# owl-project/owlExaBrick

Measured on AMD Instinct MI355X. Metric: frames/sec at 2048^2 DVR, exajet-like, MI355X, higher is better.
Workload: dtype f32; 1 GPU; c4_exajet (seed 0xe7a0003 procedural AMR, scale 1.0): 640512000 cells / 1251000 bricks / 13349488 regions, 2048x2048 DVR, dt 0.5, alpha ramp, gradient shading on, space skipping on, frameID 0; tiling=16x16 tiles interleaved over 1 GPU(s)

## Files before the change

owlexabrick_amd/csrc/exa_kernels.hip:

```cpp
#include "exa_device.h"
#include <cfloat>
#include <type_traits>

#if EXA_BASIS_FORM == 0 && EXA_EMPTY_CELLS
#define EXA_FORM_NS form0e
#elif EXA_BASIS_FORM == 0
#define EXA_FORM_NS form0
#elif EXA_BASIS_FORM == 1 && EXA_EMPTY_CELLS
#error "empty cells are a per-corner property: the per-axis association (EXA_BASIS_FORM 1) does not apply"
#elif EXA_BASIS_FORM == 1
#define EXA_FORM_NS form1
#else
#error "EXA_BASIS_FORM is 0 (source order) or 1 (per-axis association with fused multiply-adds)"
#endif
#define EXA_F1 (EXA_BASIS_FORM == 1)
#ifndef EXA_TU_ROPE
#define EXA_TU_ROPE 0
#endif
#ifndef EXA_TU_SAMPLE
#define EXA_TU_SAMPLE 0
#endif
#ifndef EXA_TU_STREAM
#define EXA_TU_STREAM 0
#endif
// ... 1818 lines not shown
  rnd.state = __float_as_uint(baseRnd.w);
  if (j & 1u) { rnd.next(); rnd.next(); }
  const V3 wN = mk(ngAmb.x, ngAmb.y, ngAmb.z);
  const V3 vN = fabsf(wN.x) > fabsf(wN.y) ? normalize(mk(-wN.z, 0.f, wN.x)) : normalize(mk(0.f, wN.z, -wN.y));
  const V3 uN = cross(vN, wN);
  const float u1 = rnd.next(), u2 = rnd.next();
  const float rr = sqrtf(u1);
  const float theta = 2.f * 3.14159265358979323846f * u2;
  const V3 sp = mk(rr * cosf(theta), rr * sinf(theta), sqrtf(1.f - u1));
  Ray ao_ray;
  ao_ray.org = mk(posFd.x, posFd.y, posFd.z);
  ao_ray.dir = normalize((sp.x * uN + sp.y * vN) + sp.z * wN);
  ao_ray.tmin = 1e-4f; ao_ray.tmax = fs.ao.length;
  return ao_ray;
}

enum { kAoDirClasses = 24, kAoCellShift = 5 };
__device__ __forceinline__ uint32_t aoRayKey(const RenderArgs &a, uint32_t slot, V3 d)
{
  const float ax = fabsf(d.x), ay = fabsf(d.y), az = fabsf(d.z);
  const uint32_t dom = (ax >= ay && ax >= az) ? 0u : (ay >= az ? 1u : 2u);
  const uint32_t oct = (d.x < 0.f ? 1u : 0u) | (d.y < 0.f ? 2u : 0u) | (d.z < 0.f ? 4u : 0u);
  uint32_t cell;
  if (a.world == 1) {
    const uint32_t px = slot % (uint32_t)a.W, py = slot / (uint32_t)a.W;
    cell = (py >> kAoCellShift) * (((uint32_t)a.W + 31u) >> kAoCellShift) + (px >> kAoCellShift);
  } else {
    cell = slot >> 10;
  }
  return cell * kAoDirClasses + oct * 3u + dom;
}
#if !EXA_TU_ROPE
__global__ __launch_bounds__(256) void aoKeyKernel(const RenderArgs a)
{
  const unsigned numRays = 2u * a.aoCount[0];
  for (unsigned j = blockIdx.x * 256u + threadIdx.x; j < numRays; j += gridDim.x * 256u) {
    const AoRecord *r = a.aoRecs + (j >> 1);
    const Ray ray = aoRayOf(a.fs, r->posFd, r->ngAmb, r->baseRnd, j);
    const uint32_t key = min(aoRayKey(a, r->slot, ray.dir), a.aoBins - 1u);
    a.aoKeys[j] = key;
    atomicAdd(&a.aoHist[key], 1u);
  }
}
__global__ __launch_bounds__(1024) void aoScanKernel(uint32_t *hist, uint32_t numBins)
{
  __shared__ uint32_t part[1024];
  const uint32_t per = (numBins + 1023u) / 1024u;
  const uint32_t b0 = min(threadIdx.x * per, numBins), b1 = min(b0 + per, numBins);
  uint32_t sum = 0;
  for (uint32_t b = b0; b < b1; b++) sum += hist[b];
  part[threadIdx.x] = sum;
  __syncthreads();
  for (uint32_t off = 1; off < 1024u; off <<= 1) {
    const uint32_t v = threadIdx.x >= off ? part[threadIdx.x - off] : 0u;
    __syncthreads();
    part[threadIdx.x] += v;
    __syncthreads();
  }
  uint32_t run = part[threadIdx.x] - sum;
  for (uint32_t b = b0; b < b1; b++) { const uint32_t c = hist[b]; hist[b] = run; run += c; }
}
__global__ __launch_bounds__(256) void aoScatterKernel(const RenderArgs a)
{
  const unsigned numRays = 2u * a.aoCount[0];
  for (unsigned j = blockIdx.x * 256u + threadIdx.x; j < numRays; j += gridDim.x * 256u)
    a.aoOrder[atomicAdd(&a.aoHist[a.aoKeys[j]], 1u)] = j;
}
__global__ __launch_bounds__(256) void aoFinalizeKernel(const RenderArgs a)
{
  const unsigned numHits = a.aoCount[0];
  for (unsigned h = blockIdx.x * 256u + threadIdx.x; h < numHits; h += gridDim.x * 256u) {
    const AoRecord *r = a.aoRecs + h;
    const float4 posFd = r->posFd, ngAmb = r->ngAmb, baseRnd = r->baseRnd;
    const uint32_t slot = r->slot;
    const int hitCnt = (int)a.aoHit[2u * h] + (int)a.aoHit[2u * h + 1u];
    const float shadow = (float)hitCnt / 2;
    const float fd = posFd.w;
    const float ns = 1.f - shadow;
    const float t_hit = a.surf[slot].w;
    a.surf[slot] = make_float4(ngAmb.w + baseRnd.x * fd * ns, ngAmb.w + baseRnd.y * fd * ns, ngAmb.w + baseRnd.z * fd * ns, t_hit);
  }
}

#endif

template <bool ISO_ONLY, bool SORTED>
__global__ __launch_bounds__(kKdBlock, (ISO_ONLY ? EXA_AO_ISO_WAVES : EXA_PREPASS_WAVES)) void aoRaysKdKernel(const RenderArgs a)
{
  static_assert(ldsFits(kdLds(1), ISO_ONLY ? EXA_AO_ISO_WAVES : EXA_PREPASS_WAVES), "LDS per workgroup x waves per SIMD exceeds the CU's 160 KB");
  const LdsPtrs lds = carveLds(kdLds(a.numXfChannels));
  Ctx<0> C;
  kernelPrologue(C, a, lds);
  float *stackF = lds.stackF, *qT = lds.qT;
  int *qRegion = lds.qRegion;
  C.fastSampler = a.fastSampler != 0;
  const ExaHipFrameState &fs = a.fs;
  const unsigned numRays = 2u * a.aoCount[0];
  for (;;) {
    unsigned base = 0;
    if ((threadIdx.x & 63) == 0) base = atomicAdd(&a.aoCount[2], 64u);
    base = (unsigned)__shfl((int)base, 0, 64);
    if (base >= numRays) break;
    const unsigned k = base + (threadIdx.x & 63);
    const bool live = k < numRays;
    const unsigned j = (SORTED && live) ? a.aoOrder[k] : k;
    int hitFlag = 0;
    float4 posFd = make_float4(0.f, 0.f, 0.f, 0.f), ngAmb = posFd, baseRnd = posFd;
    uint32_t slot = 0;
    if (live) {
      const AoRecord *r = a.aoRecs + (j >> 1);
      posFd = r->posFd; ngAmb = r->ngAmb; baseRnd = r->baseRnd; slot = r->slot;
      const Ray ao_ray = aoRayOf(fs, posFd, ngAmb, baseRnd, j);
      SurfaceHit ao;
      traceSurfacesKd<0, ISO_ONLY>(C, ao_ray, ao, false, stackF, qRegion, qT);
      if (ao.primID >= 0 || ao.primID == EXA_PRIMID_ISOSURFACE || ao.primID == EXA_PRIMID_PLANE
          || ao.primID == EXA_PRIMID_STREAMLINE) hitFlag = 1;
      if (SORTED) a.aoHit[j] = (uint8_t)hitFlag;
    }
    if (SORTED) continue;
    const int other = __shfl_xor(hitFlag, 1, 64);
    if (live && !(j & 1u)) {
      const int hitCnt = hitFlag + other;
      const float shadow = (float)hitCnt / 2;
      const float fd = posFd.w;
      const float ns = 1.f - shadow;
      const float t_hit = a.surf[slot].w;
      a.surf[slot] = make_float4(ngAmb.w + baseRnd.x * fd * ns, ngAmb.w + baseRnd.y * fd * ns, ngAmb.w + baseRnd.z * fd * ns, t_hit);
    }
  }
  if (C.guardTripped) atomicExch(a.errorFlag, 1);
}

constexpr int marchWaves(int MULTI, int STATS, bool SMALL, int NCH, bool ROPE)
{
  return NCH > 1 ? (NCH == 2 ? EXA_IL2_WAVES : EXA_IL34_WAVES)
             : (MULTI == 1 ? EXA_MULTI_WAVES
                           : (MULTI ? 5 : ((ROPE && !STATS && SMALL && EXA_BASIS_FORM == 1) ? EXA_ROPE_WAVES : EXA_MARCH_WAVES)));
}

template <bool GRAD, bool FAST, int MULTI, bool SURF, int STATS, bool SMALL, int NCH = 0, bool ROPE = false>
__global__ __launch_bounds__(kKdBlock, marchWaves(MULTI, STATS, SMALL, NCH, ROPE)) void renderFrameKdKernel(const RenderArgs a)
{
  constexpr bool CUBE = NCH == 1;
  constexpr int IL = CUBE ? 0 : NCH;
  static_assert(!CUBE || (MULTI == 0 && ROPE && SMALL && STATS == 0 && EXA_BASIS_FORM == 1 && !EXA_EMPTY_CELLS),
                "the cube records are a variant of the shipped one-channel 32-bit rope march");
#ifndef EXA_CUBE_LEAN
#define EXA_CUBE_LEAN 0
#endif
#ifndef EXA_MARCH_DEFER
#define EXA_MARCH_DEFER 1
#endif
  constexpr bool DEFER = CUBE && EXA_MARCH_DEFER;
  constexpr bool LEAN = marchWaves(MULTI, STATS, SMALL, NCH, ROPE) >= 7 && (!CUBE || EXA_CUBE_LEAN || (DEFER && GRAD));
  constexpr int PACKED_CT = !ROPE ? -1 : (STATS == 1 ? 0 : (SMALL ? 1 : -1));
  const bool packedRec = PACKED_CT < 0 ? a.leafBeginBits != 0 : PACKED_CT != 0;
  static_assert(IL == 0 || (MULTI == 2 && STATS == 0), "the interleaved march is a multi-channel variant of the shipped kernel");
  constexpr int KS = marchLds(MULTI == 1, false, 0).stackEntries;
  constexpr int QN = marchLds(MULTI == 1, ROPE, 0).queueEntries;
  static_assert(ldsFits(marchLds(MULTI == 1, ROPE, IL ? IL : (MULTI ? 2 : 1)), marchWaves(MULTI, STATS, SMALL, NCH, ROPE)),
                "LDS per workgroup x waves per SIMD exceeds the CU's 160 KB: shorten the queue or lower the occupancy");
  const LdsPtrs lds = carveLds(marchLds(MULTI == 1, ROPE, a.numXfChannels));
  float4 *queue4 = lds.queue4;
  float *stackF = lds.stackF, *qT = lds.qT;
  int *qRegion = lds.qRegion;
  for (int i = threadIdx.x; i < a.numXfChannels * EXA_NUM_XF_VALUES; i += kKdBlock) lds.xf[i] = a.xf[i];
  __syncthreads();
  Ctx<STATS> C;
  initCtx(C, a, lds);
  const unsigned long long clockBegin = clock64();
  if (STATS) for (int i = 0; i < ST_COUNT; i++) C.st[i] = 0;
  __shared__ unsigned long long lapMarks[STATS == 2 ? 8 * (kKdBlock / 64) : 1];
  if (STATS == 2) {
    C.lapMark = lapMarks + 8 * (threadIdx.x >> 6);
    if ((threadIdx.x & 63) == 0) {
      C.lapMark[0] = clock64(); C.lapMark[1] = ST_T_OTHER - ST_T_BRICK;
      for (int i = 2; i < 7; i++) C.lapMark[i] = 0;
    }
  }

  const int wavesPerBlock = kKdBlock / 64;
  const int gwave = blockIdx.x * wavesPerBlock + (threadIdx.x >> 6);
  const int tile = a.tileMap[gwave >> 2];
  const int tx = tile % a.tilesX, ty = tile / a.tilesX;
  const int wave = gwave & 3, lane = threadIdx.x & 63;
  const int inX = ((wave & 1) << 3) + laneX(lane), inY = ((wave >> 1) << 3) + laneY(lane);
  const int px = tx * kTile + inX, py = ty * kTile + inY;
  const bool inside = px < a.W && py < a.H && (a.debugPixel < 0 || a.debugPixel == px + a.W * py);

  if (STATS == 1 && a.walkProbe) C.probe = a.walkProbe + size_t(gwave) * kWalkProbeSize;
  unsigned marchIters = 0;
  if (inside) {
    const ExaHipFrameState &fs = a.fs;
    const int frameID = fs.frameID;
    Lcg rnd;
    Ray ray = cameraRay(a, px, py, rnd);
    float surface_t_hit = ray.tmax;
    if (SURF) {
      const size_t slot0 = slotOf(a, tile, inX, inY, px, py);
      surface_t_hit = a.surf[slot0].w;
      rnd.state = a.surfRnd[slot0];
    }
    const float interleavedSamplingOffset = rnd.next();
    clipToVoxelSpace(fs, ray, surface_t_hit);
    ray.org.x = __int_as_float(__builtin_amdgcn_readfirstlane(__float_as_int(ray.org.x)));
    ray.org.y = __int_as_float(__builtin_amdgcn_readfirstlane(__float_as_int(ray.org.y)));
    ray.org.z = __int_as_float(__builtin_amdgcn_readfirstlane(__float_as_int(ray.org.z)));

    Color4 pixelColor; pixelColor.x = pixelColor.y = pixelColor.z = pixelColor.w = 0.f;
    const int numChannels = a.p.numPrimaryChannels;

    KdWalk w;
    w.pk.v = 0;
    {
      Ray whole = ray; whole.tmin = -INFINITY; whole.tmax = INFINITY;
      float r0, r1;
      const bool hit = boxTest(whole, mk(a.kdLo), mk(a.kdHi), r0, r1);
      w.tn = fmaxf(r0, ray.tmin);
      w.tf = fminf(r1, ray.tmax);
      w.tEnd = w.tf;
      w.ref = (hit && w.tn < w.tf) ? (ROPE ? a.ropeRoot : a.kdMarchRoot) : EXA_KD_DONE;
    }
    bool ropeFast = false;
    if (ROPE) ropeFast = a.ropeFastDiv != 0 && !anyLane(!ropeRayInRange(ray));

    float walkTmin = ray.tmin;

    bool haveSeg = false;
    int listBegin = 0, listSize = 0;
    float flcw = 1.f;
    float t1 = 0.f, t_i = 0.f, t_sample = 0.f, actual_dt = 0.f;
    int child = 0, chan = 0;
    int4 hb0 = make_int4(0, 0, 0, 1), hb1 = make_int4(1, 1, 1, 0);
    Basis B;
    B.sumWV = 0.f; B.sumW = 0.f; B.sumD = mk(0.f, 0.f, 0.f); B.sumDC = mk(0.f, 0.f, 0.f);
    float xWV[IL > 1 ? IL - 1 : 1];
    V3 xD[IL > 1 ? IL - 1 : 1];
#pragma unroll
    for (int c = 0; c < (IL > 1 ? IL - 1 : 1); c++) { xWV[c] = 0.f; xD[c] = mk(0.f, 0.f, 0.f); }
    const float *field0 = a.sc.scalars + a.sc.channelOffset[0];
    const float *field = field0;
    float xfRcpRange0 = 0.f, xfRange0 = 0.f;
    if (FAST && !MULTI) {
      xfRange0 = __int_as_float(__builtin_amdgcn_readfirstlane(__float_as_int((fs.xfDomain[0][1] - fs.xfDomain[0][0]) + 1e-20f)));
      xfRcpRange0 = __int_as_float(__builtin_amdgcn_readfirstlane(__float_as_int(__builtin_amdgcn_rcpf(xfRange0))));
    }
    float xfRcpRangeN[IL ? IL : 1], xfRangeN[IL ? IL : 1];
#pragma unroll
    for (int c = 0; c < (IL ? IL : 1); c++) {
      xfRangeN[c] = (FAST && IL) ? __int_as_float(__builtin_amdgcn_readfirstlane(__float_as_int((fs.xfDomain[c][1] - fs.xfDomain[c][0]) + 1e-20f))) : 0.f;
      xfRcpRangeN[c] = (FAST && IL) ? __int_as_float(__builtin_amdgcn_readfirstlane(__float_as_int(__builtin_amdgcn_rcpf(xfRangeN[c])))) : 0.f;
    }

    bool pending = false;
    float pendDt = 0.f, pendFlcw = 1.f;
    auto shadePending = [&]() {
      if (B.sumW > 1e-20f) {
        const float cellValue = fdivExact<FAST>(B.sumWV, B.sumW);
        V3 grad = mk(0.f, 0.f, 0.f);
        if (GRAD) grad = gradOf(B.sumW, B.sumWV, B.sumD, B.sumDC);
        integrateVolume<FAST, STATS, (FAST && !MULTI), LEAN>(C, ray, pixelColor, pendDt, cellValue, grad, pendFlcw, 0, xfRcpRange0, xfRange0);
      }
      B.sumWV = 0.f; B.sumW = 0.f; B.sumD = mk(0.f, 0.f, 0.f); B.sumDC = mk(0.f, 0.f, 0.f);
      pending = false;
    };

    unsigned iter = 0;
    for (;; iter++) {
      if (iter == 0xfffffff0u) { C.guardTripped = true; break; }
      if (anyLane(!haveSeg && w.pk.get(PK_QCOUNT) == 0 && w.ref != EXA_KD_DONE)) {
        C.lap(ST_T_WALK);
        do {
          const bool want = w.pk.get(PK_QCOUNT) < QN && w.ref != EXA_KD_DONE;
          if (want) {
            if (ROPE) ropeStep<STATS, SMALL, QN, LEAN, PACKED_CT>(C, w, walkTmin, a, queue4, ray, ropeFast, interleavedSamplingOffset);
            else kdStep<false, STATS, SMALL, KS>(C, w, walkTmin, a, stackF, qRegion, qT, ray, 0, walkTmin, 1.f, a.kdMarchNodes, a.kdMarchRoot);
          }
        } while (anyLane(!haveSeg && w.pk.get(PK_QCOUNT) == 0 && w.ref != EXA_KD_DONE));
      }
      if (!haveSeg) {
        C.lap(ST_T_SEG);
        const int qc = w.pk.get(PK_QCOUNT);
        if (qc == 0) break;
        const int qh = w.pk.get(PK_QHEAD);
        int region;
        float t0, tiQueued = 0.f;
        if (ROPE) {
          const float4 e = queue4[qh * kKdBlock];
          region = __float_as_int(e.x); t1 = e.y; tiQueued = e.z; t0 = e.w;
        } else {
          region = qRegion[qh * kKdBlock];
          t0 = qT[(2 * qh) * kKdBlock];
          t1 = qT[(2 * qh + 1) * kKdBlock];
        }
        w.pk.template incWrap<QN>(PK_QHEAD);
        w.pk.dec(PK_QCOUNT);
        if (packedRec) {
          const unsigned d = (unsigned)region;
          listBegin = (int)(d & ((1u << a.leafBeginBits) - 1u));
          listSize = (int)((d >> a.leafBeginBits) & ((1u << a.leafSizeBits) - 1u)) + 1;
          flcw = __int_as_float((127 + (int)(d >> (a.leafBeginBits + a.leafSizeBits))) << 23);
        } else {
          const RegionInfo ri = a.sc.regionInfo[region];
          listBegin = ri.listBegin; listSize = ri.listSize;
          flcw = ri.finestLevelCellWidth;
        }
        C.count(ST_SEGMENTS);
        haveSeg = true;
        w.pk.setBit(PK_NEEDHDR);
        if (ROPE && packedRec)
          t_i = tiQueued;
        else if (a.invDtPow2 != 0.f)
          t_i = firstSampleTPow2(t0, a.p.dt * flcw, a.invDtPow2 * __int_as_float(0x7f000000 - __float_as_int(flcw)), interleavedSamplingOffset);
        else
          t_i = firstSampleT(t0, a.p.dt * flcw, interleavedSamplingOffset);
        {
          const float t_next = fminf(t_i, t1);
          t_sample = 0.5f * (fminf(t1, t_next) + t0);
          actual_dt = t_next - t0;
        }
        C.count(ST_SAMPLE_EVALS);
      }

      C.lap(ST_T_BRICK);
      C.phase(ST_W_BRICK);
      if (listSize > 1 || w.pk.get(PK_NEEDHDR)) {
        if (CUBE) {
          hb0 = *reinterpret_cast<const int4 *>(reinterpret_cast<const char *>(a.leafHdrCube) + ((uint32_t)(listBegin + child) << 4));
        } else if (SMALL) {
          const char *hp = reinterpret_cast<const char *>(a.sc.leafHdr) + ((uint32_t)(listBegin + child) << 5);
          hb0 = *reinterpret_cast<const int4 *>(hp); hb1 = *reinterpret_cast<const int4 *>(hp + 16);
        } else {
          const unsigned at = 2u * (unsigned)(listBegin + child);
          hb0 = a.sc.leafHdr[at]; hb1 = a.sc.leafHdr[at + 1u];
        }
        w.pk.clearField(PK_NEEDHDR);
      }
      if (DEFER) {
        bool ended = false;
        addBasisFast<GRAD, STATS, SMALL, false, CUBE>(C, B, hb0, hb1, field0, rayAt(ray.org, t_sample, ray.dir), a.cubeLog2, [&]() {
          if (pending) {
            shadePending();
            ended = pixelColor.w >= EXA_TERMINATION_THRESHOLD;
          }
          return !ended;
        });
        if (ended) {
          pixelColor.x = pixelColor.x * pixelColor.w;
          pixelColor.y = pixelColor.y * pixelColor.w;
          pixelColor.z = pixelColor.z * pixelColor.w;
          pixelColor.w = 1.f;
          break;
        }
        child++;
        if (child < listSize) continue;
        child = 0;
        pending = true; pendDt = actual_dt; pendFlcw = flcw;
        const float t_last = fminf(t_i, t1);
        if (t_last >= t1) {
          haveSeg = false;
          continue;
        }
        t_i += a.p.dt * flcw;
        {
          const float t_next = fminf(t_i, t1);
          t_sample = 0.5f * (fminf(t1, t_next) + t_last);
          actual_dt = t_next - t_last;
        }
        continue;
      }
      if (IL) addBasisFastIl<GRAD, SMALL, (IL ? IL : 2)>(B, xWV, xD, hb0, hb1, a.cellsIl, rayAt(ray.org, t_sample, ray.dir));
      else if (CUBE) addBasisFast<GRAD, STATS, SMALL, false, CUBE>(C, B, hb0, hb1, field0, rayAt(ray.org, t_sample, ray.dir), a.cubeLog2);
      else addBasisFast<GRAD, STATS, SMALL>(C, B, hb0, hb1, MULTI ? field : field0, rayAt(ray.org, t_sample, ray.dir));
      child++;
      if (child < listSize) continue;

      C.lap(ST_T_FINAL);
      C.phase(ST_W_FINAL);
      if (IL) {
        if (B.sumW > 1e-20f) {
#pragma unroll
          for (int c = 0; c < IL; c++) {
            const float wv = c == 0 ? B.sumWV : xWV[c == 0 ? 0 : c - 1];
            const V3 sd = c == 0 ? B.sumD : xD[c == 0 ? 0 : c - 1];
            const float cellValue = fdivExact<FAST>(wv, B.sumW);
            V3 grad = mk(0.f, 0.f, 0.f);
            if (GRAD) grad = gradOf(B.sumW, wv, sd, B.sumDC);
            integrateVolume<FAST, STATS, FAST>(C, ray, pixelColor, actual_dt, cellValue, grad, flcw, c, xfRcpRangeN[c], xfRangeN[c]);
          }
        }
#pragma unroll
        for (int c = 0; c < (IL > 1 ? IL - 1 : 1); c++) { xWV[c] = 0.f; xD[c] = mk(0.f, 0.f, 0.f); }
      } else if (B.sumW > 1e-20f) {
        C.count(ST_SAMPLES);
        const float cellValue = fdivExact<FAST>(B.sumWV, B.sumW);
        V3 grad = mk(0.f, 0.f, 0.f);
        if (GRAD) grad = gradOf(B.sumW, B.sumWV, B.sumD, B.sumDC);
        integrateVolume<FAST, STATS, (FAST && !MULTI), LEAN>(C, ray, pixelColor, actual_dt, cellValue, grad, flcw, MULTI ? chan : 0, xfRcpRange0, xfRange0);
      }
      B.sumWV = 0.f; B.sumW = 0.f; B.sumD = mk(0.f, 0.f, 0.f); B.sumDC = mk(0.f, 0.f, 0.f);
      child = 0;
      if (MULTI && !IL) {
        chan++;
        if (chan < numChannels) {
          field = a.sc.scalars + a.sc.channelOffset[chan];
          C.count(ST_SAMPLE_EVALS);
          continue;
        }
        chan = 0; field = field0;
      }
      if (pixelColor.w >= EXA_TERMINATION_THRESHOLD) {
        pixelColor.x = pixelColor.x * pixelColor.w;
        pixelColor.y = pixelColor.y * pixelColor.w;
        pixelColor.z = pixelColor.z * pixelColor.w;
        pixelColor.w = 1.f;
        break;
      }
      const float t_last = fminf(t_i, t1);
      if (t_last >= t1) {
        haveSeg = false;
        continue;
      }
      t_i += a.p.dt * flcw;
      {
        const float t_next = fminf(t_i, t1);
        t_sample = 0.5f * (fminf(t1, t_next) + t_last);
        actual_dt = t_next - t_last;
      }
      C.count(ST_SAMPLE_EVALS);
    }

    if (DEFER && pending) {
      shadePending();
      if (pixelColor.w >= EXA_TERMINATION_THRESHOLD) {
        pixelColor.x = pixelColor.x * pixelColor.w;
        pixelColor.y = pixelColor.y * pixelColor.w;
        pixelColor.z = pixelColor.z * pixelColor.w;
        pixelColor.w = 1.f;
      }
    }
    C.lap(ST_T_OTHER);
    marchIters = iter;
    size_t slot, colorSlot;
    {
      unsigned tid = threadIdx.x, bid = blockIdx.x;
      asm volatile("" : "+v"(tid));
      asm volatile("" : "+s"(bid));
      const int lane2 = tid & 63, wave2 = (tid >> 6) & 3;
      const int inX2 = ((wave2 & 1) << 3) + laneX(lane2), inY2 = ((wave2 >> 1) << 3) + laneY(lane2);
      slot = (a.world == 1) ? size_t(tx * kTile + inX2) + size_t(a.W) * (ty * kTile + inY2)
                            : size_t(a.tileMap[(bid * wavesPerBlock + (tid >> 6)) >> 2] / a.world) * kTilePixels + (inY2 * kTile + inX2);
      colorSlot = a.colorRowMajor ? size_t(tx * kTile + inX2) + size_t(a.W) * (ty * kTile + inY2) : slot;
    }
    if (SURF && a.pixOut) {
      a.pixOut[slot] = make_float4(pixelColor.x, pixelColor.y, pixelColor.z, pixelColor.w);
    } else {
    float4 bgColor = make_float4(0.f, 0.f, 0.f, 0.f);
    if (SURF) bgColor = a.surf[slot];
    float cr = pixelColor.w * pixelColor.x + (1.f - pixelColor.w) * bgColor.x;
    float cg = pixelColor.w * pixelColor.y + (1.f - pixelColor.w) * bgColor.y;
    float cb = pixelColor.w * pixelColor.z + (1.f - pixelColor.w) * bgColor.z;
    if (fs.clockScale > 0.f) cr = clockHeat(fs.clockScale, clockBegin);
    if (frameID > 0) {
      const float4 acc = a.accum[slot];
      cr += acc.x; cg += acc.y; cb += acc.z;
    }
    a.accum[slot] = make_float4(cr, cg, cb, 1.f);
    const float div = frameID + 1.f;
    cr = cr / div; cg = cg / div; cb = cb / div;
    a.color[colorSlot] = make_rgba8(linear_to_srgb(cr), linear_to_srgb(cg), linear_to_srgb(cb));
    }
  }

  if (a.tileCost) {
    unsigned v = marchIters;
    for (int off = 32; off > 0; off >>= 1) v = max(v, (unsigned)__shfl_down((int)v, off, 64));
    unsigned bid = blockIdx.x, tid = threadIdx.x;
    asm volatile("" : "+s"(bid));
    asm volatile("" : "+v"(tid));
    if (lane == 0) atomicMax(&a.tileCost[a.tileMap[(bid * wavesPerBlock + (tid >> 6)) >> 2]], v);
  }
  if (C.guardTripped) atomicExch(a.errorFlag, 1);
  if (STATS == 2) {
    if (lane < 5 && C.lapMark[2 + lane]) atomicAdd(&a.stats[ST_T_BRICK + lane], C.lapMark[2 + lane]);
  }
  if (STATS == 1) {
    for (int i = 0; i < ST_COUNT; i++) {
      unsigned long long v = inside ? C.st[i] : 0ull;
      for (int off = 32; off > 0; off >>= 1) v += __shfl_down(v, off, 64);
      if ((threadIdx.x & 63) == 0 && v) atomicAdd(&a.stats[i], v);
    }
    __shared__ unsigned wgMaxIters;
    if (threadIdx.x == 0) wgMaxIters = 0;
    __syncthreads();
    unsigned v = marchIters;
    for (int off = 32; off > 0; off >>= 1) v = max(v, (unsigned)__shfl_down((int)v, off, 64));
    if (lane == 0) atomicMax(&wgMaxIters, v);
    __syncthreads();
    if (lane == 0) atomicAdd(&a.stats[ST_WAVE_ITERS], (unsigned long long)v);
    if (threadIdx.x == 0) atomicAdd(&a.stats[ST_TILE_ITERS], 4ull * wgMaxIters);
  }
}

__device__ __forceinline__ void kdCollectStep(Ctx<0> &C, KdWalk &w, const float winLo, const float winHi, const RenderArgs &a,
                                              float *stackF, const Ray &ray, const KdNodeDev *nodes, const int root,
                                              float4 *out, unsigned &count)
{
  if (w.ref != EXA_KD_EMPTY && !(w.tn < winHi)) { w.ref = EXA_KD_DONE; return; }
  if (w.ref < 0 && w.ref > EXA_KD_DONE) {
    if (w.tn >= winLo && w.tn < w.tf) out[count++] = make_float4(__int_as_float(~w.ref), w.tn, w.tf, 0.f);
    w.ref = EXA_KD_EMPTY;
  }
  if (w.ref == EXA_KD_EMPTY || (w.ref != EXA_KD_DONE && !(w.tf > winLo))) kdPop(C, w, root, stackF, nodes, ray);
  if (w.ref < 0 || !(w.tf > winLo) || !(w.tn < winHi)) return;
  kdNodeStage<kKdStackEntries, false, 0>(C, w, stackF, ray, nodes, 2);
}

template <bool GRAD, bool FAST, bool SURF, int L, bool SMALL>
__global__ __launch_bounds__(kKdBlock, 4) void renderFrameKdWideKernel(const RenderArgs a)
{
  static_assert(ldsFits(kdLds(1), 4), "LDS per workgroup x waves per SIMD exceeds the CU's 160 KB");
  const LdsPtrs lds = carveLds(kdLds(a.numXfChannels));
  float *stackF = lds.stackF;
  Ctx<false> C;
  kernelPrologue(C, a, lds);
  const unsigned long long clockBegin = clock64();

  __builtin_amdgcn_s_setprio(3);
  const int tile = a.wideTileMap[blockIdx.x / L];
  const int part = blockIdx.x % L;
  const int tx = tile % a.tilesX, ty = tile / a.tilesX;
  const int lane = threadIdx.x & 63, sub = lane & (L - 1), lead = lane & ~(L - 1);
  const bool leader = sub == 0;
  const int r = part * (kTilePixels / L) + (threadIdx.x >> 6) * (64 / L) + lane / L;
  const int inX = (((r >> 6) & 1) << 3) + (r & 7), inY = ((r >> 7) << 3) + ((r >> 3) & 7);
  const int px = tx * kTile + inX, py = ty * kTile + inY;
  const bool inside = px < a.W && py < a.H && (a.debugPixel < 0 || a.debugPixel == px + a.W * py);

  unsigned myVisits = 0;
  if (inside) {
    const ExaHipFrameState &fs = a.fs;
    const int frameID = fs.frameID;
    Lcg rnd;
    Ray ray = cameraRay(a, px, py, rnd);
    const size_t slot = slotOf(a, tile, inX, inY, px, py);
    float surface_t_hit = ray.tmax;
    if (SURF) {
      surface_t_hit = a.surf[slot].w;
      rnd.state = a.surfRnd[slot];
    }
    const float interleavedSamplingOffset = rnd.next();
    clipToVoxelSpace(fs, ray, surface_t_hit);

    Color4 pixelColor; pixelColor.x = pixelColor.y = pixelColor.z = pixelColor.w = 0.f;

    float4 *const mySegs = a.wideSegs + (size_t(blockIdx.x / L) * kTilePixels * L + size_t(r) * L + sub) * kWideSegCap;
    unsigned myCount = 0;
    KdWalk w;
    w.pk.v = 0;
    float winLo, winHi;
    {
      Ray whole = ray; whole.tmin = -INFINITY; whole.tmax = INFINITY;
      float r0, r1;
      const bool hit = boxTest(whole, mk(a.kdLo), mk(a.kdHi), r0, r1);
      w.tn = fmaxf(r0, ray.tmin);
      w.tf = fminf(r1, ray.tmax);
      w.tEnd = w.tf;
      w.ref = (hit && w.tn < w.tf) ? a.kdMarchRoot : EXA_KD_DONE;
      const float span = w.tf - w.tn;
      winLo = sub == 0 ? -INFINITY : w.tn + span * (float(sub) / float(L));
      winHi = sub == L - 1 ? INFINITY : w.tn + span * (float(sub + 1) / float(L));
      for (unsigned g = 0;; g++) {
        if (g == 0xfffffff0u) { C.guardTripped = true; break; }
        const bool want = w.ref != EXA_KD_DONE && myCount < kWideSegCap;
        if (!anyLane(want)) break;
        if (want) kdCollectStep(C, w, winLo, winHi, a, stackF, ray, a.kdMarchNodes, a.kdMarchRoot, mySegs, myCount);
      }
    }
    __builtin_amdgcn_fence(__ATOMIC_RELEASE, "wavefront");
    __builtin_amdgcn_fence(__ATOMIC_ACQUIRE, "wavefront");
    float walkTmin = ray.tmin;
    int curWin = 0;
    unsigned curIdx = 0, curCount = (unsigned)__shfl((int)myCount, lead, 64);
    const float4 *curSegs = a.wideSegs + (size_t(blockIdx.x / L) * kTilePixels * L + size_t(r) * L) * kWideSegCap;

    bool haveSeg = false, newStep = false, needHdr = false, mine = false;
    int listBegin = 0, listSize = 0;
    float flcw = 1.f, dtSeg = 0.f;
    float t1 = 0.f, tiBase = 0.f, tlBase = 0.f;
    float t_sample = 0.f, actual_dt = 0.f;
    int child = 0;
    int4 hb0 = make_int4(0, 0, 0, 1), hb1 = make_int4(1, 1, 1, 0);
    Basis B;
    B.sumWV = 0.f; B.sumW = 0.f; B.sumD = mk(0.f, 0.f, 0.f); B.sumDC = mk(0.f, 0.f, 0.f);
    const float *field0 = a.sc.scalars + a.sc.channelOffset[0];

    for (unsigned iter = 0;; iter++) {
      if (iter == 0xfffffff0u) { C.guardTripped = true; break; }
      if (!haveSeg) {
        int region = -1;
        float t0 = 0.f;
        for (;;) {
          if (curIdx >= curCount) {
            const bool mineIsCur = sub == curWin;
            if (__shfl((int)(w.ref != EXA_KD_DONE), lead + curWin, 64)) {
              if (mineIsCur) {
                myCount = 0;
                for (unsigned g = 0; w.ref != EXA_KD_DONE && myCount < kWideSegCap; g++) {
                  if (g == 0xfffffff0u) { C.guardTripped = true; break; }
                  kdCollectStep(C, w, winLo, winHi, a, stackF, ray, a.kdMarchNodes, a.kdMarchRoot, mySegs, myCount);
                }
              }
              __builtin_amdgcn_fence(__ATOMIC_RELEASE, "wavefront");
              __builtin_amdgcn_fence(__ATOMIC_ACQUIRE, "wavefront");
              curIdx = 0;
              curCount = (unsigned)__shfl((int)myCount, lead + curWin, 64);
              continue;
            }
            if (++curWin == L) break;
            curIdx = 0;
            curCount = (unsigned)__shfl((int)myCount, lead + min(curWin, L - 1), 64);
            curSegs += kWideSegCap;
            continue;
          }
          const float4 e = curSegs[curIdx++];
          t0 = fmaxf(walkTmin, e.y);
          if (t0 < e.z) {
            region = __float_as_int(e.x);
            t1 = e.z;
            walkTmin = t1 * (1.0000001f);
            break;
          }
        }
        if (curWin == L) break;
        if (a.leafBeginBits) {
// ... 116 lines not shown
  const int tx = tile % a.tilesX, ty = tile / a.tilesX;
  const int inX = threadIdx.x & 15, inY = threadIdx.x >> 4;
  const int px = tx * kTile + inX, py = ty * kTile + inY;
  if (!(px < a.W && py < a.H) || !(a.debugPixel < 0 || a.debugPixel == px + a.W * py)) return;
  const size_t slot = slotOf(a, tile, inX, inY, px, py);
  const size_t colorSlot = a.colorRowMajor ? size_t(px) + size_t(a.W) * py : slot;
  const float4 pixelColor = a.pixOut[slot];
  const float4 bgColor = a.surf[slot];
  const int frameID = a.fs.frameID;
  float cr = pixelColor.w * pixelColor.x + (1.f - pixelColor.w) * bgColor.x;
  float cg = pixelColor.w * pixelColor.y + (1.f - pixelColor.w) * bgColor.y;
  float cb = pixelColor.w * pixelColor.z + (1.f - pixelColor.w) * bgColor.z;
  if (frameID > 0) {
    const float4 acc = a.accum[slot];
    cr += acc.x; cg += acc.y; cb += acc.z;
  }
  a.accum[slot] = make_float4(cr, cg, cb, 1.f);
  const float div = frameID + 1.f;
  cr = cr / div; cg = cg / div; cb = cb / div;
  a.color[colorSlot] = make_rgba8(linear_to_srgb(cr), linear_to_srgb(cg), linear_to_srgb(cb));
}
hipError_t launchCompositeKd(const RenderArgs &a, int numBlocks, hipStream_t s)
{
  if (numBlocks <= 0) return hipSuccess;
  hipLaunchKernelGGL(compositeKdKernel, dim3(numBlocks), dim3(256), 0, s, a);
  return hipGetLastError();
}

hipError_t launchRenderKdWide(const RenderArgs &a, int numTiles, int lanesPerRay, bool grad, bool fast, bool surf, hipStream_t s)
{
  if (numTiles <= 0) return hipSuccess;
#if EXA_EMPTY_CELLS
  return hipErrorNotSupported;
#else
  const size_t lds = kdLds(a.numXfChannels).total;
  const dim3 grid(numTiles * lanesPerRay), block(kKdBlock);
  const bool small = a.mul24 && a.addr32;
#define EXA_W4(G, F, S, L) do { if (small) hipLaunchKernelGGL((renderFrameKdWideKernel<G, F, S, L, true>), grid, block, lds, s, a); \
                                else hipLaunchKernelGGL((renderFrameKdWideKernel<G, F, S, L, false>), grid, block, lds, s, a); } while (0)
#define EXA_W3(G, F, S) do { if (lanesPerRay == 2) EXA_W4(G, F, S, 2); else EXA_W4(G, F, S, 4); } while (0)
#define EXA_W2(G, F) do { if (surf) EXA_W3(G, F, true); else EXA_W3(G, F, false); } while (0)
  if (grad) { if (fast) EXA_W2(true, true); else EXA_W2(true, false); }
  else      { if (fast) EXA_W2(false, true); else EXA_W2(false, false); }
#undef EXA_W4
#undef EXA_W2
#undef EXA_W3
  return hipGetLastError();
#endif
}

static bool isoOnly(const RenderArgs &a)
{
  bool only = a.numTris == 0 && a.numStreamPrims == 0;
  for (int i = 0; i < EXA_MAX_CONTOUR_PLANES; i++) only = only && !a.fs.contour[i].enabled;
  return only;
}

hipError_t launchSurfacePrepassKd(const RenderArgs &a, int numBlocks, bool stats, hipStream_t s)
{
  if (numBlocks <= 0) return hipSuccess;
  const size_t lds = kdLds(a.numXfChannels).total;
  const dim3 grid(numBlocks * (256 / kKdBlock)), block(kKdBlock);
  const bool defer = !stats && a.aoRecs && a.aoCount;
  if (stats)        hipLaunchKernelGGL((surfacePrepassKdKernel<1, false, false>), grid, block, lds, s, a);
  else if (isoOnly(a)) { if (defer) hipLaunchKernelGGL((surfacePrepassKdKernel<0, true, true>), grid, block, lds, s, a);
                      else       hipLaunchKernelGGL((surfacePrepassKdKernel<0, true, false>), grid, block, lds, s, a); }
  else              { if (defer) hipLaunchKernelGGL((surfacePrepassKdKernel<0, false, true>), grid, block, lds, s, a);
                      else       hipLaunchKernelGGL((surfacePrepassKdKernel<0, false, false>), grid, block, lds, s, a); }
  return hipGetLastError();
}

hipError_t launchAoRaysKd(const RenderArgs &a, int numBlocks, hipStream_t s)
{
  if (numBlocks <= 0) return hipSuccess;
  const size_t lds = kdLds(a.numXfChannels).total;
  const dim3 block(kKdBlock);
  const bool iso = isoOnly(a);
  const bool defer = a.aoRecs && a.aoCount;
  if (defer && a.fs.ao.enabled) {
    const int maxBlocks = 256 * (iso ? EXA_AO_ISO_WAVES : EXA_PREPASS_WAVES);
    const long long upper = ((long long)numBlocks * kTilePixels * 2 + kKdBlock - 1) / kKdBlock;
    const dim3 g2((unsigned)(upper < maxBlocks ? upper : maxBlocks));
    if (a.aoKeys) {
      const dim3 gs((unsigned)(upper < 2048 ? upper : 2048)), b256(256);
      if (hipError_t e = hipMemsetAsync(a.aoHist, 0, size_t(a.aoBins) * sizeof(uint32_t), s)) return e;
      hipLaunchKernelGGL(aoKeyKernel, gs, b256, 0, s, a);
      hipLaunchKernelGGL(aoScanKernel, dim3(1), dim3(1024), 0, s, a.aoHist, a.aoBins);
      hipLaunchKernelGGL(aoScatterKernel, gs, b256, 0, s, a);
      if (iso) hipLaunchKernelGGL((aoRaysKdKernel<true, true>), g2, block, lds, s, a);
      else         hipLaunchKernelGGL((aoRaysKdKernel<false, true>), g2, block, lds, s, a);
      hipLaunchKernelGGL(aoFinalizeKernel, gs, b256, 0, s, a);
    } else {
      if (iso) hipLaunchKernelGGL((aoRaysKdKernel<true, false>), g2, block, lds, s, a);
      else         hipLaunchKernelGGL((aoRaysKdKernel<false, false>), g2, block, lds, s, a);
    }
  }
  return hipGetLastError();
}

#endif

template <bool ROPE>
static hipError_t launchRenderKdT(const RenderArgs &a, int numBlocks, bool grad, bool fast, bool surf, int stats, hipStream_t s)
{
  if (numBlocks <= 0) return hipSuccess;
#ifndef EXA_LDS_PAD
#define EXA_LDS_PAD 0
#endif
  const int mode = a.p.numPrimaryChannels > 1 ? ((a.numXfChannels <= 2 && !stats) ? 1 : 2) : 0;
  const dim3 grid(numBlocks * (256 / kKdBlock)), block(kKdBlock);
  const bool small = a.mul24 && a.addr32 && (!ROPE || (a.ropeAddr32 && a.leafBeginBits));
#define EXA_LAUNCH(G, F, M, I, S, A) hipLaunchKernelGGL((renderFrameKdKernel<G, F, M, I, S, A, 0, ROPE>), grid, block, \
                                                        marchLds((M) == 1, ROPE, a.numXfChannels, EXA_LDS_PAD).total, s, a)
#define EXA_PICK2(G, F, M, I) do { if (stats == 1) EXA_LAUNCH(G, F, (M ? 2 : 0), I, 1, false); else if (stats == 2) EXA_LAUNCH(G, F, (M ? 2 : 0), I, 2, false); \
                                   else if (small) EXA_LAUNCH(G, F, M, I, 0, true); else EXA_LAUNCH(G, F, M, I, 0, false); } while (0)
#define EXA_PICK(G, F, M) do { if (surf) EXA_PICK2(G, F, M, true); else EXA_PICK2(G, F, M, false); } while (0)
#define EXA_PICKM(G, F) do { if (mode == 0) EXA_PICK(G, F, 0); else if (mode == 1) EXA_PICK(G, F, 1); else EXA_PICK(G, F, 2); } while (0)
#if !EXA_EMPTY_CELLS
  const int nch = (a.cellsIl && !stats && a.p.numPrimaryChannels >= 2 && a.p.numPrimaryChannels <= 4) ? a.p.numPrimaryChannels : 0;
  if (nch) {
    const bool smallIl = small && a.il32;
#define EXA_IL4(G, F, I, A, N) hipLaunchKernelGGL((renderFrameKdKernel<G, F, 2, I, 0, A, N, ROPE>), grid, block, \
                                                  marchLds(false, ROPE, a.numXfChannels, EXA_LDS_PAD).total, s, a)
#define EXA_IL3(G, F, I, A) do { if (nch == 2) EXA_IL4(G, F, I, A, 2); else if (nch == 3) EXA_IL4(G, F, I, A, 3); else EXA_IL4(G, F, I, A, 4); } while (0)
#define EXA_IL2(G, F, I) do { if (smallIl) EXA_IL3(G, F, I, true); else EXA_IL3(G, F, I, false); } while (0)
#define EXA_IL1(G, F) do { if (surf) EXA_IL2(G, F, true); else EXA_IL2(G, F, false); } while (0)
    if (grad) { if (fast) EXA_IL1(true, true); else EXA_IL1(true, false); }
    else      { if (fast) EXA_IL1(false, true); else EXA_IL1(false, false); }
#undef EXA_IL1
#undef EXA_IL2
#undef EXA_IL3
#undef EXA_IL4
    return hipGetLastError();
  }
#endif
#if EXA_TU_ROPE && EXA_BASIS_FORM == 1 && !EXA_EMPTY_CELLS
  if (ROPE && mode == 0 && !stats && small && fast && a.leafHdrCube) {
#define EXA_CUBE(G, I) hipLaunchKernelGGL((renderFrameKdKernel<G, true, 0, I, 0, true, 1, ROPE>), grid, block, \
                                          marchLds(false, ROPE, a.numXfChannels, EXA_LDS_PAD).total, s, a)
    if (grad) { if (surf) EXA_CUBE(true, true); else EXA_CUBE(true, false); }
    else      { if (surf) EXA_CUBE(false, true); else EXA_CUBE(false, false); }
#undef EXA_CUBE
    return hipGetLastError();
  }
#endif
  if (grad) { if (fast) EXA_PICKM(true, true); else EXA_PICKM(true, false); }
  else      { if (fast) EXA_PICKM(false, true); else EXA_PICKM(false, false); }
#undef EXA_PICKM
#undef EXA_PICK
#undef EXA_PICK2
#undef EXA_LAUNCH
  return hipGetLastError();
}
#if EXA_TU_ROPE
hipError_t launchRenderKdRope(const RenderArgs &a, int numBlocks, bool grad, bool fast, bool surf, int stats, hipStream_t s)
{ return launchRenderKdT<true>(a, numBlocks, grad, fast, surf, stats, s); }
#else
hipError_t launchRenderKd(const RenderArgs &a, int numBlocks, bool grad, bool fast, bool surf, int stats, hipStream_t s)
{ return launchRenderKdT<false>(a, numBlocks, grad, fast, surf, stats, s); }
#endif

}

#if EXA_BASIS_FORM == 0 && !EXA_EMPTY_CELLS && !EXA_TU_ROPE
using namespace form0;
__global__ __launch_bounds__(256) void kdRefitKernel(KdNodeDev *nodes, KdNodeDev *marchNodes, const int32_t *nodeIds, int count,
                                                     const uint8_t *active, int which)
{
  const int i = blockIdx.x * 256 + threadIdx.x;
  if (i >= count) return;
  const int id = nodeIds[i];
  const KdNodeDev n = nodes[id];
  const int sh = 2 + 2 * which;
  auto act = [&](int ref) -> uint32_t {
    if (ref == EXA_KD_EMPTY) return 0u;
    if (ref < 0) return active[~ref] ? 1u : 0u;
    return ((nodes[ref].word >> sh) & 3u) ? 1u : 0u;
  };
  const uint32_t bits = act(n.left) | (act(n.right) << 1);
  const uint32_t word = (n.word & ~(3u << sh)) | (bits << sh);
  nodes[id].word = word;
  if (marchNodes) marchNodes[id].word = word;
}

hipError_t launchKdRefit(KdNodeDev *nodes, KdNodeDev *marchNodes, const int32_t *nodeIds, int count, const uint8_t *active, int which, hipStream_t s)
{
  if (count <= 0) return hipSuccess;
  hipLaunchKernelGGL(kdRefitKernel, dim3((count + 255) / 256), dim3(256), 0, s, nodes, marchNodes, nodeIds, count, active, which);
  return hipGetLastError();
}

__global__ __launch_bounds__(256) void ropeActivityKernel(RopeLeaf *leaves, uint32_t numRegions, const uint8_t *active, int which, uint32_t *activeCount)
{
  const uint32_t r = blockIdx.x * 256u + threadIdx.x;
  const bool act = r < numRegions && active[r] != 0;
  if (leaves && r < numRegions) {
    const uint32_t f = leaves[r].flags;
    leaves[r].flags = (f & ~(1u << which)) | ((act ? 1u : 0u) << which);
  }
  if (activeCount) {
    const unsigned long long m = __ballot(act);
    if ((threadIdx.x & 63) == 0 && m) atomicAdd(activeCount, (uint32_t)__popcll(m));
  }
}
hipError_t launchRopeActivity(RopeLeaf *leaves, uint32_t numRegions, const uint8_t *active, int which, uint32_t *activeCount, hipStream_t s)
{
  if (numRegions == 0) return hipSuccess;
  hipLaunchKernelGGL(ropeActivityKernel, dim3((numRegions + 255) / 256), dim3(256), 0, s, leaves, numRegions, active, which, activeCount);
  return hipGetLastError();
}
#endif

#if !EXA_TU_ROPE
namespace EXA_FORM_NS {

__device__ __forceinline__ bool sampleDirection(Ctx<false> &C, V3 pos, V3 &result)
{
  Ray ray; ray.org = pos; ray.dir = mk(1.f, 1.f, 1.f); ray.tmin = 0.f; ray.tmax = 2e-10f;
  const RegionHit prd = traceRegion(C, C.a->volNodes, ray);
  result = mk(0.f, 0.f, 0.f);
  if (prd.leafID < 0) return false;
  const RegionInfo ri = C.a->sc.regionInfo[prd.leafID];
  V3 unused;
  float r0 = 0.f, r1 = 0.f, r2 = 0.f;
  bool ok = samplePoint<false, false>(C, r0, unused, ri, pos, C.a->tracerChannels[0]);
  if (ok) ok = samplePoint<false, false>(C, r1, unused, ri, pos, C.a->tracerChannels[1]);
  if (ok) ok = samplePoint<false, false>(C, r2, unused, ri, pos, C.a->tracerChannels[2]);
  result = mk(r0, r1, r2);
  return ok;
}

__global__ __launch_bounds__(256) void computeTracesKernel(const RenderArgs a, float *traces, int count)
{
  __shared__ int stackLds[kStackDepth * 256];
  const int i = blockIdx.x * 256 + threadIdx.x;
  Ctx<false> C;
  C.a = &a; C.xfLds = nullptr; C.stack = stackLds + threadIdx.x; C.guardTripped = false;
  if (i >= count) return;
  const int t = a.timestep, NT = a.numTimesteps;
  if (!(t < NT)) return;
  V3 p = mk(traces + 3 * (size_t(i) * NT + (t - 1)));
  const V3 pp = p;
  if (p.x < 2e10f) {
    bool valid = true;
    V3 k1, k2, k3, k4;
    valid &= sampleDirection(C, p, k1);
    k1 = a.steplen * k1;
    const V3 ptry1 = p + .5f * k1;
    valid &= sampleDirection(C, ptry1, k2);
    k2 = a.steplen * k2;
    const V3 ptry2 = p + .5f * k2;
    valid &= sampleDirection(C, ptry2, k3);
    k3 = a.steplen * k3;
    const V3 ptry3 = p + k3;
    valid &= sampleDirection(C, ptry3, k4);
    k4 = a.steplen * k4;
    p = p + (1 / 6.f) * (((k1 + 2.f * k2) + 2.f * k3) + k4);
    const bool inside = p.x >= a.worldLo[0] && p.y >= a.worldLo[1] && p.z >= a.worldLo[2]
                     && p.x <= a.worldHi[0] && p.y <= a.worldHi[1] && p.z <= a.worldHi[2];
    if (!valid || !inside || length(p - pp) < 1e-10f) p = mk(2e10f, 2e10f, 2e10f);
  }
  float *dst = traces + 3 * (size_t(i) * NT + t);
  dst[0] = p.x; dst[1] = p.y; dst[2] = p.z;
}

hipError_t launchComputeTraces(const RenderArgs &a, float *traces, int count, hipStream_t s)
{
  if (count <= 0) return hipSuccess;
  hipLaunchKernelGGL(computeTracesKernel, dim3((count + 255) / 256), dim3(256), 0, s, a, traces, count);
  return hipGetLastError();
}

}
#endif

#if EXA_BASIS_FORM == 0 && !EXA_EMPTY_CELLS && !EXA_TU_ROPE
__global__ __launch_bounds__(256) void volumeActivityKernel(DeviceScene sc, ExaHipFrameState fs, ExaHipParams p,
                                                            const float4 *xf, uint8_t *active, float tfFracMagic)
{
  extern __shared__ __attribute__((aligned(16))) unsigned char smem[];
  float4 *xfLds = reinterpret_cast<float4 *>(smem);
  for (int i = threadIdx.x; i < p.numChannels * EXA_NUM_XF_VALUES; i += 256) xfLds[i] = xf[i];
  __syncthreads();
  const uint32_t r = blockIdx.x * 256u + threadIdx.x;
  if (r >= sc.numRegions) return;
  const float2 vr = sc.valueRange[r];
  bool act = false;
  for (int c = 0; c < p.numChannels && !act; ++c) {
    const float dlo = fs.xfDomain[c][0], dhi = fs.xfDomain[c][1];
    if (vr.x > dhi) continue;
    if (vr.y < dlo) continue;
    const float scaled_lo = (vr.x - dlo) / ((dhi - dlo) + 1e-20f);
    const float scaled_hi = (vr.y - dlo) / ((dhi - dlo) + 1e-20f);
    const int idx_lo = min(EXA_NUM_XF_VALUES - 1, max(0, int(scaled_lo * (EXA_NUM_XF_VALUES - 1))));
    const int idx_hi = min(EXA_NUM_XF_VALUES - 1, max(0, int(scaled_hi * (EXA_NUM_XF_VALUES - 1)) + 1));
    for (int i = idx_lo; i <= idx_hi; i++) {
      float cellValue = float(i) / (EXA_NUM_XF_VALUES - 1);
      cellValue *= dhi - dlo;
      cellValue += dlo;
      const Color4 rgba = lookupXF(xfLds, fs, cellValue, c, tfFracMagic);
      if (rgba.w > 0.f) { act = true; break; }
    }
  }
  active[r] = (uint8_t)(p.spaceSkippingEnabled ? (act ? 1 : 0) : 1);
}

// ... 162 lines not shown
```

Measured before the change: 66.11 frames/s.

## Cut live registers in cube march by reloading late kernel args and split LEAN

For the cube-record rope kernel, the epilogue now re-reads kernel arguments through a fresh kernarg-segment pointer (hidden behind an opaque zero), recomputes tile coordinates from tileMap, and keeps the clock start in LDS. This stops SGPRs/VGPRs holding args, tile indices and the 64-bit clock from staying live across the whole march loop. The LEAN option is split so the rope walk and the shading integration can be leaned independently (default: integration only). The aim is lower register pressure to hold occupancy, at the cost of a few extra scalar loads, an LDS write/read, and tile recomputation in the epilogue.

```diff
diff --git a/owlexabrick_amd/csrc/exa_kernels.hip b/owlexabrick_amd/csrc/exa_kernels.hip
--- a/owlexabrick_amd/csrc/exa_kernels.hip
+++ b/owlexabrick_amd/csrc/exa_kernels.hip
@@ -1994,7 +1994,12 @@
 #define EXA_MARCH_DEFER 1
 #endif
   constexpr bool DEFER = CUBE && EXA_MARCH_DEFER;
-  constexpr bool LEAN = marchWaves(MULTI, STATS, SMALL, NCH, ROPE) >= 7 && (!CUBE || EXA_CUBE_LEAN || (DEFER && GRAD));
+#ifndef EXA_CUBE_GRAD_LEAN
+#define EXA_CUBE_GRAD_LEAN 1
+#endif
+  constexpr bool LEAN7 = marchWaves(MULTI, STATS, SMALL, NCH, ROPE) >= 7;
+  constexpr bool LEAN = LEAN7 && (!CUBE || EXA_CUBE_LEAN || ((EXA_CUBE_GRAD_LEAN & 1) && DEFER && GRAD));
+  constexpr bool LEAN_WALK = LEAN7 && (!CUBE || EXA_CUBE_LEAN || ((EXA_CUBE_GRAD_LEAN & 2) && DEFER && GRAD));
   constexpr int PACKED_CT = !ROPE ? -1 : (STATS == 1 ? 0 : (SMALL ? 1 : -1));
   const bool packedRec = PACKED_CT < 0 ? a.leafBeginBits != 0 : PACKED_CT != 0;
   static_assert(IL == 0 || (MULTI == 2 && STATS == 0), "the interleaved march is a multi-channel variant of the shipped kernel");
@@ -2012,7 +2017,8 @@
   initCtx(C, a, lds);
   const unsigned long long clockBegin = clock64();
   if (STATS) for (int i = 0; i < ST_COUNT; i++) C.st[i] = 0;
-  __shared__ unsigned long long lapMarks[STATS == 2 ? 8 * (kKdBlock / 64) : 1];
+  __shared__ unsigned long long lapMarks[STATS == 2 ? 8 * (kKdBlock / 64) : (CUBE ? kKdBlock / 64 : 1)];
+  if constexpr (CUBE) lapMarks[threadIdx.x >> 6] = clockBegin;
   if (STATS == 2) {
     C.lapMark = lapMarks + 8 * (threadIdx.x >> 6);
     if ((threadIdx.x & 63) == 0) {
@@ -2028,13 +2034,19 @@
   const int wave = gwave & 3, lane = threadIdx.x & 63;
   const int inX = ((wave & 1) << 3) + laneX(lane), inY = ((wave >> 1) << 3) + laneY(lane);
   const int px = tx * kTile + inX, py = ty * kTile + inY;
-  const bool inside = px < a.W && py < a.H && (a.debugPixel < 0 || a.debugPixel == px + a.W * py);
+  const bool inside = CUBE ? bool(int(px < a.W) & int(py < a.H) & (int(a.debugPixel < 0) | int(a.debugPixel == px + a.W * py)))
+                           : (px < a.W && py < a.H && (a.debugPixel < 0 || a.debugPixel == px + a.W * py));
 
   if (STATS == 1 && a.walkProbe) C.probe = a.walkProbe + size_t(gwave) * kWalkProbeSize;
   unsigned marchIters = 0;
+  using LateArgs = std::conditional_t<CUBE, const __attribute__((address_space(4))) RenderArgs, const RenderArgs>;
+  LateArgs *late;
+  if constexpr (!CUBE) late = &a;
+#define LATE_ARGS() do { if constexpr (CUBE) {  \
+    unsigned zero; asm volatile("s_mov_b32 %0, 0" : "=s"(zero)); \
+    late = (LateArgs *)((const __attribute__((address_space(4))) char *)__builtin_amdgcn_kernarg_segment_ptr() + zero); } } while (0)
   if (inside) {
     const ExaHipFrameState &fs = a.fs;
-    const int frameID = fs.frameID;
     Lcg rnd;
     Ray ray = cameraRay(a, px, py, rnd);
     float surface_t_hit = ray.tmax;
@@ -2115,7 +2127,7 @@
         do {
           const bool want = w.pk.get(PK_QCOUNT) < QN && w.ref != EXA_KD_DONE;
           if (want) {
-            if (ROPE) ropeStep<STATS, SMALL, QN, LEAN, PACKED_CT>(C, w, walkTmin, a, queue4, ray, ropeFast, interleavedSamplingOffset);
+            if (ROPE) ropeStep<STATS, SMALL, QN, LEAN_WALK, PACKED_CT>(C, w, walkTmin, a, queue4, ray, ropeFast, interleavedSamplingOffset);
             else kdStep<false, STATS, SMALL, KS>(C, w, walkTmin, a, stackF, qRegion, qT, ray, 0, walkTmin, 1.f, a.kdMarchNodes, a.kdMarchRoot);
           }
         } while (anyLane(!haveSeg && w.pk.get(PK_QCOUNT) == 0 && w.ref != EXA_KD_DONE));
@@ -2284,45 +2296,60 @@
     C.lap(ST_T_OTHER);
     marchIters = iter;
     size_t slot, colorSlot;
+    LATE_ARGS();
+    unsigned tid2;
     {
       unsigned tid = threadIdx.x, bid = blockIdx.x;
       asm volatile("" : "+v"(tid));
       asm volatile("" : "+s"(bid));
+      tid2 = tid;
       const int lane2 = tid & 63, wave2 = (tid >> 6) & 3;
       const int inX2 = ((wave2 & 1) << 3) + laneX(lane2), inY2 = ((wave2 >> 1) << 3) + laneY(lane2);
-      slot = (a.world == 1) ? size_t(tx * kTile + inX2) + size_t(a.W) * (ty * kTile + inY2)
-                            : size_t(a.tileMap[(bid * wavesPerBlock + (tid >> 6)) >> 2] / a.world) * kTilePixels + (inY2 * kTile + inX2);
-      colorSlot = a.colorRowMajor ? size_t(tx * kTile + inX2) + size_t(a.W) * (ty * kTile + inY2) : slot;
-    }
-    if (SURF && a.pixOut) {
-      a.pixOut[slot] = make_float4(pixelColor.x, pixelColor.y, pixelColor.z, pixelColor.w);
+      int tx2 = tx, ty2 = ty;
+      if constexpr (CUBE) {
+        const int tile2 = late->tileMap[(bid * wavesPerBlock + __builtin_amdgcn_readfirstlane(tid >> 6)) >> 2];
+        tx2 = tile2 % late->tilesX; ty2 = tile2 / late->tilesX;
+      }
+      slot = (late->world == 1) ? size_t(tx2 * kTile + inX2) + size_t(late->W) * (ty2 * kTile + inY2)
+                            : size_t(late->tileMap[(bid * wavesPerBlock + (tid >> 6)) >> 2] / late->world) * kTilePixels + (inY2 * kTile + inX2);
+      colorSlot = late->colorRowMajor ? size_t(tx2 * kTile + inX2) + size_t(late->W) * (ty2 * kTile + inY2) : slot;
+    }
+    if (SURF && late->pixOut) {
+      late->pixOut[slot] = make_float4(pixelColor.x, pixelColor.y, pixelColor.z, pixelColor.w);
     } else {
     float4 bgColor = make_float4(0.f, 0.f, 0.f, 0.f);
-    if (SURF) bgColor = a.surf[slot];
+    if (SURF) bgColor = late->surf[slot];
     float cr = pixelColor.w * pixelColor.x + (1.f - pixelColor.w) * bgColor.x;
     float cg = pixelColor.w * pixelColor.y + (1.f - pixelColor.w) * bgColor.y;
     float cb = pixelColor.w * pixelColor.z + (1.f - pixelColor.w) * bgColor.z;
-    if (fs.clockScale > 0.f) cr = clockHeat(fs.clockScale, clockBegin);
+    if (late->fs.clockScale > 0.f) {
+      unsigned long long begin = clockBegin;
+      if constexpr (CUBE) begin = lapMarks[tid2 >> 6];
+      cr = clockHeat(late->fs.clockScale, begin);
+    }
+    const int frameID = late->fs.frameID;
     if (frameID > 0) {
-      const float4 acc = a.accum[slot];
+      const float4 acc = late->accum[slot];
       cr += acc.x; cg += acc.y; cb += acc.z;
     }
-    a.accum[slot] = make_float4(cr, cg, cb, 1.f);
+    late->accum[slot] = make_float4(cr, cg, cb, 1.f);
     const float div = frameID + 1.f;
     cr = cr / div; cg = cg / div; cb = cb / div;
-    a.color[colorSlot] = make_rgba8(linear_to_srgb(cr), linear_to_srgb(cg), linear_to_srgb(cb));
-    }
-  }
-
-  if (a.tileCost) {
+    late->color[colorSlot] = make_rgba8(linear_to_srgb(cr), linear_to_srgb(cg), linear_to_srgb(cb));
+    }
+  }
+
+  LATE_ARGS();
+  if (late->tileCost) {
     unsigned v = marchIters;
     for (int off = 32; off > 0; off >>= 1) v = max(v, (unsigned)__shfl_down((int)v, off, 64));
     unsigned bid = blockIdx.x, tid = threadIdx.x;
     asm volatile("" : "+s"(bid));
     asm volatile("" : "+v"(tid));
-    if (lane == 0) atomicMax(&a.tileCost[a.tileMap[(bid * wavesPerBlock + (tid >> 6)) >> 2]], v);
-  }
-  if (C.guardTripped) atomicExch(a.errorFlag, 1);
+    if (lane == 0) atomicMax(&late->tileCost[late->tileMap[(bid * wavesPerBlock + (tid >> 6)) >> 2]], v);
+  }
+  if (C.guardTripped) atomicExch(late->errorFlag, 1);
+#undef LATE_ARGS
   if (STATS == 2) {
     if (lane < 5 && C.lapMark[2 + lane]) atomicAdd(&a.stats[ST_T_BRICK + lane], C.lapMark[2 + lane]);
   }
@@ -2745,6 +2772,22 @@
 #undef EXA_LAUNCH
   return hipGetLastError();
 }
+#if EXA_TU_ROPE && EXA_BASIS_FORM == 1 && !EXA_EMPTY_CELLS
+#if EXA_CUBE_LEAN
+#define EXA_CUBE_GRAD_LEAN_BUILT 3
+#else
+#define EXA_CUBE_GRAD_LEAN_BUILT (EXA_MARCH_DEFER ? EXA_CUBE_GRAD_LEAN : 0)
+#endif
+#if EXA_CUBE_GRAD_LEAN_BUILT == 0
+extern "C" __device__ __attribute__((used)) const int exa_cube_grad_lean_0 = 0;
+#elif EXA_CUBE_GRAD_LEAN_BUILT == 1
+extern "C" __device__ __attribute__((used)) const int exa_cube_grad_lean_1 = 1;
+#elif EXA_CUBE_GRAD_LEAN_BUILT == 2
+extern "C" __device__ __attribute__((used)) const int exa_cube_grad_lean_2 = 2;
+#else
+extern "C" __device__ __attribute__((used)) const int exa_cube_grad_lean_3 = 3;
+#endif
+#endif
 #if EXA_TU_ROPE
 hipError_t launchRenderKdRope(const RenderArgs &a, int numBlocks, bool grad, bool fast, bool surf, int stats, hipStream_t s)
 { return launchRenderKdT<true>(a, numBlocks, grad, fast, surf, stats, s); }
```

After: 66.76 frames/s, median of 6. No clear change (+1.0%).
